# merijn-23/magr-ray-tracer

Hardware: AMD Instinct MI355X
Metric: Mrays/sec + extend-kernel HBM GB/s, sponza 1080p 256spp (higher is better)
Workload: dtype f32

## Files before the change

### include/rt355.h

```cpp
#ifndef RT355_H
#define RT355_H
#include "rt355_types.h"

#ifdef __cplusplus
extern "C" {
#endif

#define RT_OK            0
#define RT_E_INVALID    (-1)
#define RT_E_DEVICE     (-2)
#define RT_E_NOMEM      (-3)
#define RT_E_UNSUPPORTED (-4)

#define RT_SHADING_SIMPLE       0
#define RT_SHADING_NEE          1
#define RT_SAMPLING_HEMISPHERE  0
#define RT_SAMPLING_COSINE      1
#define RT_ACCEL_BVH2           0
#define RT_ACCEL_BVH4           1

typedef struct RtCtx RtCtx;

typedef struct RtConfig {
    int32_t width, height;
// ... 84 lines not shown
int rt_debug_sbvh_phases(float* out);
int rt_build_bvh4(int32_t device, const RtBVHNode2* nodes2, int32_t nNodes, int32_t nIdx, const uint32_t* roots, int32_t nRoots,
                  RtBVHNode4* out4, RtBvh4Stats* stats);

typedef struct RtUpdateStats {
    double  gpu_ms;
    int32_t prims, nodes;
    int32_t tlas_nodes, tlas_depth;
    int32_t reconfigured;
    int32_t reserved[3];
} RtUpdateStats;
int rt_update_scene(RtCtx* ctx, const RtPrimitive* prims, int32_t first, int32_t count, const RtBVHInstance* blas, int32_t nBlas,
                    RtUpdateStats* stats);
#define RT_REBUILD_SAH   0
#define RT_REBUILD_LBVH  1
#define RT_REBUILD_SBVH  2
typedef struct RtRebuildStats {
    double  gpu_ms;
    double  wall_ms;
    double  stage_ms, build_ms, derive_ms, tlas_ms, commit_ms;
    int32_t prims, blas_built;
    int32_t nodes, n_idx;
    int32_t max_depth;
    int32_t tlas_nodes, tlas_depth;
    int32_t reconfigured;
    int32_t spatial_splits, prims_clipped;
} RtRebuildStats;
int rt_rebuild_scene(RtCtx* ctx, const RtPrimitive* prims, int32_t first, int32_t count, const RtBVHInstance* blas, int32_t nBlas,
                     int32_t builder, const RtBuildOptions* opts, RtRebuildStats* stats);
int rt_debug_rebuild_allocations(RtCtx* ctx, int64_t* count);
int rt_blas_ranges(const RtBVHNode2* nodes, int32_t nNodes, const uint32_t* primIdx, int32_t nIdx, int32_t nPrims,
                   const RtBVHInstance* blas, int32_t nBlas, int32_t* firstOut, int32_t* countOut);
#define RT_SCENE_PRIMS         0
#define RT_SCENE_BVH           1
#define RT_SCENE_TLAS          2
#define RT_SCENE_INSTANCES     3
#define RT_SCENE_PAIRS         4
#define RT_SCENE_TRI_RECS      5
#define RT_SCENE_SHADE_RECS    6
#define RT_SCENE_LIGHT_RECS    7
#define RT_SCENE_TLAS_PAIRS    8
#define RT_SCENE_TLAS_PAIRS_P  9
#define RT_SCENE_INST_RECS    10
#define RT_SCENE_QUADS        11
#define RT_SCENE_ROOT_ENTRY   12
#define RT_SCENE_BVH2_KEPT    13
int rt_debug_get_scene_array(RtCtx* ctx, int32_t which, void* out, int64_t capacityBytes, int64_t* bytes);

typedef struct RtGroup RtGroup;
int rt_group_create(const RtConfig* cfg, int32_t lanes, RtGroup** out);
int rt_group_destroy(RtGroup* g);
int rt_group_lanes(RtGroup* g);
int rt_group_concurrency(RtGroup* g);
RtCtx* rt_group_lane(RtGroup* g, int32_t m);
uint64_t rt_group_frames(RtGroup* g);
int rt_group_upload_scene(RtGroup* g,
                          const RtPrimitive* prims, int32_t nPrims, const RtMaterial* mats, int32_t nMats,
                          const RtFloat4* textures, int32_t nTexels, const uint32_t* lights, int32_t nLights,
                          const void* bvhNodes, int32_t nNodes, const uint32_t* primIdx, int32_t nIdx,
                          const RtTLASNode* tlas, int32_t nTlas, const RtBVHInstance* blas, int32_t nBlas);
int rt_group_upload_scene_bvh2(RtGroup* g,
                               const RtPrimitive* prims, int32_t nPrims, const RtMaterial* mats, int32_t nMats,
                               const RtFloat4* textures, int32_t nTexels, const uint32_t* lights, int32_t nLights,
                               const RtBVHNode2* bvhNodes, int32_t nNodes, const uint32_t* primIdx, int32_t nIdx,
                               const RtTLASNode* tlas, int32_t nTlas, const RtBVHInstance* blas, int32_t nBlas);
int rt_group_share_scene(RtGroup* g, RtGroup* from);
int rt_group_update_scene(RtGroup* g, const RtPrimitive* prims, int32_t first, int32_t count, const RtBVHInstance* blas, int32_t nBlas,
                          RtUpdateStats* stats);
int rt_group_rebuild_scene(RtGroup* g, const RtPrimitive* prims, int32_t first, int32_t count, const RtBVHInstance* blas, int32_t nBlas,
                           int32_t builder, const RtBuildOptions* opts, RtRebuildStats* stats);
int rt_group_seed(RtGroup* g, uint64_t firstStream);
int rt_group_reset(RtGroup* g);
int rt_group_render(RtGroup* g, const RtCamera* cam, const RtSettings* settings, int32_t frames);
int rt_group_synchronize(RtGroup* g);
int rt_group_sum(RtGroup* g, void* devicePtr);
int rt_group_read_accum(RtGroup* g, RtFloat4* out);
int rt_group_focus(RtGroup* g, int32_t x, int32_t y, const RtCamera* cam, float* t);
int rt_group_postproc(RtGroup* g, int32_t frames, float vignette, float gamma, float chromatic, RtFloat4* outF32, uint8_t* outRGBA8);

int rt_set_seeds(RtCtx* ctx, const uint32_t* seeds, int64_t n);
int rt_seed_default(RtCtx* ctx);
int rt_get_seeds(RtCtx* ctx, uint32_t* out, int64_t n);

int rt_bind_accum(RtCtx* ctx, void* devicePtr);
void* rt_accum_device_ptr(RtCtx* ctx);
void* rt_stream(RtCtx* ctx);

int rt_reset(RtCtx* ctx);

int rt_render(RtCtx* ctx, const RtCamera* cam, const RtSettings* settings, int32_t frames);
int rt_synchronize(RtCtx* ctx);

int rt_focus(RtCtx* ctx, int32_t x, int32_t y, const RtCamera* cam, float* t);

int rt_read_accum(RtCtx* ctx, RtFloat4* out);
int rt_write_accum(RtCtx* ctx, const RtFloat4* in);
int rt_read_counters(RtCtx* ctx, RtCounters* out);
int rt_reset_counters(RtCtx* ctx);
int rt_set_profile(RtCtx* ctx, int32_t level);
int rt_read_stage_times(RtCtx* ctx, RtStageTimes* out);
int rt_reset_stage_times(RtCtx* ctx);

int rt_postproc(RtCtx* ctx, int32_t frames, float vignette, float gamma, float chromatic, RtFloat4* outF32, uint8_t* outRGBA8);

int rt_stage_begin_frame(RtCtx* ctx);
int rt_stage_generate(RtCtx* ctx, const RtCamera* cam, const RtSettings* s);
// ... 31 lines not shown
```

### magr_ray_tracer_amd/_lib.py

```python
import ctypes as C
import os

import numpy as np

_PKG = os.path.dirname(os.path.abspath(__file__))

f4 = np.dtype((np.float32, 4))
Ray = np.dtype([("O", f4), ("D", f4), ("rD", f4), ("N", f4), ("I", f4), ("intensity", f4), ("t", "<f4"),
                ("primIdx", "<i4"), ("bounces", "<i4"), ("pixelIdx", "<i4"), ("inside", "u1"), ("lastSpecular", "u1"),
                ("_pad0", "u1", 2), ("u", "<f4"), ("v", "<f4"), ("_pad1", "<u4")], align=False)
ShadowRay = np.dtype([("I", f4), ("L", f4), ("Nl", f4), ("intensity", f4), ("BRDF", f4), ("lightIdx", "<i4"),
                      ("pixelIdx", "<i4"), ("dotNL", "<f4"), ("dist", "<f4")])
Material = np.dtype([("color", f4), ("absorption", f4), ("specular", "<f4"), ("n1", "<f4"), ("n2", "<f4"),
                     ("isDielectric", "u1"), ("_pad0", "u1", 3), ("texIdx", "<i4"), ("texW", "<i4"), ("texH", "<i4"),
                     ("isLight", "u1"), ("_pad1", "u1", 3), ("emittance", f4)])
Primitive = np.dtype([("v0", f4), ("v1", f4), ("v2", f4), ("N", f4), ("centroid", f4), ("uv0", "<f4", 2), ("uv1", "<f4", 2),
                      ("uv2", "<f4", 2), ("_padt", "<f4", 2), ("objType", "<i4"), ("matIdx", "<i4"), ("area", "<f4"),
                      ("_pad", "<u4")])
Camera = np.dtype([("type", "<i4"), ("fov", "<f4"), ("aperture", "<f4"), ("focalLength", "<f4"), ("forward", f4),
                   ("right", f4), ("up", f4), ("origin", f4), ("horizontal", f4), ("vertical", f4), ("topLeft", f4)])
Settings = np.dtype([("numPrimitives", "<i4"), ("numLights", "<i4"), ("tracerType", "<i4"), ("frames", "<i4"),
                     ("antiAliasing", "<i4"), ("numInRays", "<i4"), ("numOutRays", "<i4"), ("shadowRays", "<i4"),
                     ("renderBVH", "<i4"), ("focalLength", "<f4")])
BVHNode2 = np.dtype([("aabbMin", f4), ("aabbMax", f4), ("first", "<u4"), ("count", "<u4"), ("_pad", "<u4", 2)])
# ... 21 lines not shown
                     [("sah_cost", "<f4"), ("device_ms", "<f4"), ("wall_ms", "<f4"), ("peak_refs", "<i4")])
Bvh4Stats = np.dtype([(n, "<i4") for n in ("live_nodes", "levels", "stack_need", "largest_leaf")] + [("device_ms", "<f4"), ("wall_ms", "<f4")])
KernelInfo = np.dtype([(n, "<i4") for n in ("layout", "persist", "persist4", "stack_entries", "persist_grid", "persist_grid_connect",
                                             "shade_grid", "n_blas")])

_SIZES = {"Ray": (Ray, 128), "ShadowRay": (ShadowRay, 96), "Material": (Material, 80), "Primitive": (Primitive, 128),
          "Camera": (Camera, 128), "Settings": (Settings, 40), "BVHNode2": (BVHNode2, 48), "BVHNode4": (BVHNode4, 160),
          "BVHInstance": (BVHInstance, 68), "TLASNode": (TLASNode, 48), "BuildOptions": (BuildOptions, 16), "BuildStats": (BuildStats, 32), "SbvhStats": (SbvhStats, 48), "Bvh4Stats": (Bvh4Stats, 24), "ShadowRecord": (ShadowRecord, 48), "Config": (Config, 64)}
for _n, (_d, _s) in _SIZES.items():
    assert _d.itemsize == _s, (_n, _d.itemsize, _s)

SHADING_SIMPLE, SHADING_NEE = 0, 1
SAMPLING_HEMISPHERE, SAMPLING_COSINE = 0, 1
ACCEL_BVH2, ACCEL_BVH4 = 0, 1
PRIM_SPHERE, PRIM_PLANE, PRIM_TRIANGLE = 0, 1, 2
MATH_EXP, MATH_SIN, MATH_COS, MATH_ACOS, MATH_ATAN, MATH_F2I, MATH_ATAN2, MATH_SPHERE_TEXEL, MATH_NORMALIZE4, MATH_LENGTH4 = range(10)
MATH_WORDS = {MATH_EXP: (1, 1), MATH_SIN: (1, 1), MATH_COS: (1, 1), MATH_ACOS: (1, 1), MATH_ATAN: (1, 1), MATH_F2I: (1, 1),
              MATH_ATAN2: (2, 1), MATH_SPHERE_TEXEL: (6, 2), MATH_NORMALIZE4: (4, 4), MATH_LENGTH4: (4, 1)}
MATH_SWEEP_BLOCK_BITS = 20
MAX_BOUNCES = 7
BUILTINS_DEFAULT, BUILTINS_IEEE, BUILTINS_REFERENCE = 0, 1, 2
BUILTINS = {None: BUILTINS_DEFAULT, "ieee": BUILTINS_IEEE, "reference": BUILTINS_REFERENCE}


def builtins_value(name):
    try:
        return BUILTINS[name]
    except (KeyError, TypeError):
        raise ValueError(f"builtins must be None, 'ieee' or 'reference', not {name!r}") from None


RT_OK, RT_E_INVALID, RT_E_DEVICE, RT_E_NOMEM, RT_E_UNSUPPORTED = 0, -1, -2, -3, -4
SCENE_ARRAYS = {"prims": 0, "bvh": 1, "tlas": 2, "instances": 3, "pairs": 4, "triRecs": 5, "shadeRecs": 6, "lightRecs": 7,
                "tlasPairs": 8, "tlasPairsP": 9, "instRecs": 10}
SCENE_ARRAYS_BVH4 = {"quads": 11, "rootEntry": 12, "bvh2Kept": 13}
UpdateStats = np.dtype([("gpu_ms", "<f8"), ("prims", "<i4"), ("nodes", "<i4"), ("tlas_nodes", "<i4"), ("tlas_depth", "<i4"),
                        ("reconfigured", "<i4"), ("reserved", "<i4", 3)])
assert UpdateStats.itemsize == 40
REBUILD_SAH, REBUILD_LBVH, REBUILD_SBVH = 0, 1, 2
RebuildStats = np.dtype([(n, "<f8") for n in ("gpu_ms", "wall_ms", "stage_ms", "build_ms", "derive_ms", "tlas_ms", "commit_ms")] +
                        [(n, "<i4") for n in ("prims", "blas_built", "nodes", "n_idx", "max_depth", "tlas_nodes", "tlas_depth", "reconfigured")] +
                        [("spatial_splits", "<i4"), ("prims_clipped", "<i4")])
assert RebuildStats.itemsize == 96

DEVICE_SYMBOLS = [
    "rt_last_error", "rt_device_count", "rt_kernel_info", "rt_builtins", "rt_top_levels", "rt_shade_footprint", "rt_shade_tables", "rt_create", "rt_destroy", "rt_upload_scene", "rt_share_scene", "rt_set_seeds", "rt_seed_default",
    "rt_get_seeds", "rt_bind_accum", "rt_accum_device_ptr", "rt_stream", "rt_reset", "rt_render", "rt_synchronize", "rt_focus",
    "rt_read_accum", "rt_write_accum", "rt_postproc", "rt_read_counters", "rt_reset_counters", "rt_read_stage_times", "rt_reset_stage_times", "rt_set_profile",
    "rt_stage_begin_frame", "rt_stage_generate", "rt_stage_extend", "rt_stage_shade", "rt_stage_connect",
    "rt_debug_get_rays", "rt_debug_set_rays", "rt_debug_get_shadow", "rt_debug_enable_steps", "rt_debug_get_steps", "rt_debug_math",
    "rt_debug_math_sweep", "rt_debug_math_mode", "rt_debug_math_sweep_mode", "rt_validate_scene", "rt_build_bvh2", "rt_build_bvh2_sah", "rt_debug_sah_phases", "rt_build_bvh2_sbvh", "rt_debug_sbvh_phases", "rt_update_scene", "rt_group_update_scene", "rt_debug_get_scene_array",
    "rt_rebuild_scene", "rt_group_rebuild_scene", "rt_blas_ranges", "rt_debug_rebuild_allocations",
    "rt_build_bvh4", "rt_upload_scene_bvh2", "rt_group_upload_scene_bvh2",
    "rt_group_create", "rt_group_destroy", "rt_group_lanes", "rt_group_concurrency", "rt_group_lane", "rt_group_frames", "rt_group_upload_scene", "rt_group_share_scene",
    "rt_group_seed", "rt_group_reset", "rt_group_render", "rt_group_synchronize", "rt_group_sum", "rt_group_read_accum", "rt_group_focus",
    "rt_group_postproc"]
HOST_SYMBOLS = [
    "rth_last_error", "rth_scene_create", "rth_scene_destroy", "rth_add_material", "rth_add_texture", "rth_load_texture", "rth_add_sphere",
    "rth_add_plane", "rth_add_triangle", "rth_add_quad", "rth_add_triangles", "rth_build_blas", "rth_build_bvh4",
    "rth_build_tlas", "rth_bvh4_from_nodes", "rth_set_instance_transform", "rth_primitives", "rth_materials", "rth_textures", "rth_lights",
    "rth_bvh2_nodes", "rth_bvh4_nodes", "rth_prim_idx", "rth_tlas_nodes", "rth_blas_nodes", "rth_bvh_stats", "rth_camera",
    "rth_renderer_create", "rth_renderer_destroy", "rth_renderer_init", "rth_renderer_set_camera", "rth_renderer_tick",
    "rth_renderer_read", "rth_renderer_camera", "rth_seed_stream", "rth_load_model", "rth_save_png",
    "rth_set_build_threads", "rth_renderer_save_frame", "rth_renderer_camera_move", "rth_renderer_camera_mouse", "rth_renderer_camera_zoom", "rth_renderer_frames", "rth_renderer_set_lanes", "rth_renderer_set_builtins", "rth_renderer_builtins",
    "rth_build_blas_lbvh", "rth_build_bvh2_lbvh", "rth_lbvh_stats", "rth_set_primitives", "rth_refit",
    "rth_build_blas_sah_gpu", "rth_build_bvh2_sah", "rth_build_blas_sbvh_gpu", "rth_build_bvh2_sbvh", "rth_rebuild", "rth_blas_ranges",
    "rth_build_bvh4_gpu", "rth_build_bvh4_levels"]

_dev = None
_host = None


class NativeLibraryMissing(RuntimeError):
    pass


def _load(name, local=False):
    path = os.path.join(_PKG, name)
    if not os.path.exists(path):
        raise NativeLibraryMissing(
            f"{path} is missing: build it with `python -m magr_ray_tracer_amd.build` (hipcc, gfx950). "
            "The hot path has no Python/CPU fallback.")
    return C.CDLL(path, mode=C.RTLD_LOCAL if local else C.RTLD_GLOBAL)


_variants = {}


def device_lib(variant=None):
    global _dev
    if variant:
        if variant not in _variants:
            keep, _dev = _dev, None
            try:
                _variants[variant] = _bind_device(_load(f"librt355_{variant}.so", local=True))
            finally:
                _dev = keep
        return _variants[variant]
    if _dev is None:
        _dev = _bind_device(_load("librt355.so"))
    return _dev


def _bind_device(lib):
    if True:
        vp, i32, i64 = C.c_void_p, C.c_int32, C.c_int64
        lib.rt_last_error.restype = C.c_char_p
# ... 10 lines not shown
        lib.rt_build_bvh4.argtypes = [i32, vp, i32, i32, vp, i32, vp, vp]
        lib.rt_share_scene.argtypes = [vp, vp]
        lib.rt_set_seeds.argtypes = [vp, vp, i64]
        lib.rt_seed_default.argtypes = [vp]
        lib.rt_get_seeds.argtypes = [vp, vp, i64]
        lib.rt_bind_accum.argtypes = [vp, vp]
        lib.rt_accum_device_ptr.argtypes = [vp]
        lib.rt_accum_device_ptr.restype = vp
        lib.rt_stream.argtypes = [vp]
        lib.rt_stream.restype = vp
        lib.rt_reset.argtypes = [vp]
        lib.rt_render.argtypes = [vp, vp, vp, i32]
        lib.rt_synchronize.argtypes = [vp]
        lib.rt_focus.argtypes = [vp, i32, i32, vp, C.POINTER(C.c_float)]
        lib.rt_read_accum.argtypes = [vp, vp]
        lib.rt_read_counters.argtypes = [vp, vp]
        lib.rt_write_accum.argtypes = [vp, vp]
        lib.rt_postproc.argtypes = [vp, i32, C.c_float, C.c_float, C.c_float, vp, vp]
        lib.rt_reset_counters.argtypes = [vp]
        lib.rt_read_stage_times.argtypes = [vp, vp]
        lib.rt_reset_stage_times.argtypes = [vp]
        lib.rt_set_profile.argtypes = [vp, i32]
        lib.rt_stage_begin_frame.argtypes = [vp]
        lib.rt_stage_generate.argtypes = [vp, vp, vp]
        lib.rt_stage_extend.argtypes = [vp, i32, i32]
        lib.rt_stage_shade.argtypes = [vp, i32]
        lib.rt_stage_connect.argtypes = [vp, i32, i32]
        lib.rt_debug_get_rays.argtypes = [vp, i32, vp, i32, C.POINTER(i32)]
        lib.rt_debug_set_rays.argtypes = [vp, i32, vp, i32]
        lib.rt_debug_get_shadow.argtypes = [vp, i32, i32, vp, i32, C.POINTER(i32)]
        lib.rt_debug_get_steps.argtypes = [vp, vp, i32, C.POINTER(i32)]
        lib.rt_debug_enable_steps.argtypes = [vp, i32]
        lib.rt_debug_math.argtypes = [i32, vp, vp, i64]
        lib.rt_debug_math_sweep.argtypes = [i32, i32, i32, vp]
        lib.rt_debug_math_mode.argtypes = [i32, i32, vp, vp, i64]
        lib.rt_debug_math_sweep_mode.argtypes = [i32, i32, i32, i32, vp]
        lib.rt_validate_scene.argtypes = [i32, vp, i32, vp, i32, vp, i32, vp, i32, vp, i32, vp, i32, vp, i32, vp, i32]
        lib.rt_build_bvh2.argtypes = [i32, vp, vp, i32, i32, i32, C.c_uint32, C.c_uint32, vp, i32, C.POINTER(i32), vp, vp]
        lib.rt_build_bvh2_sah.argtypes = [i32, vp, i32, i32, i32, C.c_uint32, C.c_uint32, vp, i32, C.POINTER(i32), vp, vp]
        lib.rt_debug_sah_phases.argtypes = [vp]
        lib.rt_build_bvh2_sbvh.argtypes = [i32, C.c_float, vp, i32, i32, i32, C.c_uint32, C.c_uint32, vp, i32, C.POINTER(i32), vp, i32, C.POINTER(i32), vp]
        lib.rt_debug_sbvh_phases.argtypes = [vp]
        lib.rt_update_scene.argtypes = [vp, vp, i32, i32, vp, i32, vp]
        lib.rt_group_update_scene.argtypes = [vp, vp, i32, i32, vp, i32, vp]
        lib.rt_debug_get_scene_array.argtypes = [vp, i32, vp, i64, C.POINTER(i64)]
        lib.rt_rebuild_scene.argtypes = [vp, vp, i32, i32, vp, i32, i32, vp, vp]
        lib.rt_group_rebuild_scene.argtypes = [vp, vp, i32, i32, vp, i32, i32, vp, vp]
        lib.rt_debug_rebuild_allocations.argtypes = [vp, vp]
        lib.rt_blas_ranges.argtypes = [vp, i32, vp, i32, i32, vp, i32, vp, vp]
        lib.rt_group_create.argtypes = [vp, i32, C.POINTER(vp)]
        lib.rt_group_destroy.argtypes = [vp]
        lib.rt_group_lanes.argtypes = [vp]
        lib.rt_group_concurrency.argtypes = [vp]
        lib.rt_group_lane.argtypes = [vp, i32]
        lib.rt_group_lane.restype = vp
        lib.rt_group_frames.argtypes = [vp]
        lib.rt_group_frames.restype = C.c_uint64
        lib.rt_group_upload_scene.argtypes = [vp, vp, i32, vp, i32, vp, i32, vp, i32, vp, i32, vp, i32, vp, i32, vp, i32]
        lib.rt_group_seed.argtypes = [vp, C.c_uint64]
        lib.rt_group_share_scene.argtypes = [vp, vp]
        lib.rt_group_reset.argtypes = [vp]
        lib.rt_group_render.argtypes = [vp, vp, vp, i32]
        lib.rt_group_synchronize.argtypes = [vp]
        lib.rt_group_sum.argtypes = [vp, vp]
        lib.rt_group_read_accum.argtypes = [vp, vp]
        lib.rt_group_focus.argtypes = [vp, i32, i32, vp, C.POINTER(C.c_float)]
        lib.rt_group_postproc.argtypes = [vp, i32, C.c_float, C.c_float, C.c_float, vp, vp]
    return lib


def host_lib():
    global _host
    if _host is None:
        device_lib()
        lib = _load("librt355_host.so")
        vp, i32, fp, cp = C.c_void_p, C.c_int, C.POINTER(C.c_float), C.c_char_p
        lib.rth_last_error.restype = cp
        lib.rth_scene_create.restype = vp
        lib.rth_scene_destroy.argtypes = [vp]
        lib.rth_add_material.argtypes = [vp, cp, vp]
        lib.rth_add_texture.argtypes = [vp, cp, vp, i32, i32]
        lib.rth_load_texture.argtypes = [vp, cp, cp]
        lib.rth_add_sphere.argtypes = [vp, fp, C.c_float, cp]
        lib.rth_add_plane.argtypes = [vp, fp, C.c_float, cp]
        lib.rth_add_triangle.argtypes = [vp, fp, fp, fp, fp, fp, fp, cp, i32]
        lib.rth_add_quad.argtypes = [vp, fp, fp, fp, fp, cp, i32]
        lib.rth_add_triangles.argtypes = [vp, vp, vp, i32, cp, i32]
        lib.rth_build_blas.argtypes = [vp, i32, C.c_float]
        lib.rth_build_bvh4.argtypes = [vp]
        lib.rth_build_bvh4_gpu.argtypes = [vp, i32]
        lib.rth_build_bvh4_levels.argtypes = [vp, C.c_int32, C.c_int32, vp, C.c_int32, vp, vp, vp, vp, vp]
        lib.rth_build_blas_lbvh.argtypes = [vp, i32, i32, vp]
        lib.rth_build_bvh2_lbvh.argtypes = [vp, vp, C.c_int32, C.c_int32, C.c_int32, C.c_uint32, C.c_uint32, vp, C.c_int32,
                                            C.POINTER(C.c_int32), vp, vp]
        lib.rth_lbvh_stats.argtypes = [vp, vp]
        lib.rth_build_blas_sah_gpu.argtypes = [vp, i32, i32]
        lib.rth_build_bvh2_sah.argtypes = [vp, C.c_int32, C.c_int32, C.c_int32, C.c_uint32, C.c_uint32, vp, C.c_int32,
                                           C.POINTER(C.c_int32), vp, vp]
        lib.rth_build_blas_sbvh_gpu.argtypes = [vp, i32, C.c_float, i32]
        lib.rth_build_bvh2_sbvh.argtypes = [C.c_float, vp, C.c_int32, C.c_int32, C.c_int32, C.c_uint32, C.c_uint32, vp, C.c_int32,
                                            C.POINTER(C.c_int32), vp, C.c_int32, C.POINTER(C.c_int32), vp]
        lib.rth_set_primitives.argtypes = [vp, i32, i32, vp]
        lib.rth_refit.argtypes = [vp]
        lib.rth_rebuild.argtypes = [vp, i32, vp]
        lib.rth_blas_ranges.argtypes = [vp, vp, vp]
        lib.rth_set_build_threads.argtypes = [vp, i32]
# ... 43 lines not shown
```

### magr_ray_tracer_amd/csrc/rt355.hip

```cpp
#include <hip/hip_runtime.h>
#include <hip/hip_ext.h>
#include <algorithm>
#include <chrono>
#include <cstdio>
#include <cmath>
#include <cstdlib>
#include <cstring>
#include <memory>
#include <atomic>
#include <string>
#include <vector>
#include "../../include/rt355.h"
#include "rt355_kernels.h"
#include "scene_dev.h"

using namespace rt355dev;
using namespace scenedev;

static constexpr int kAdmitAnySgpr = 6, kAdmit96Sgpr = 7;
static constexpr int kTopLevelsExtend = 6, kTopLevelsConnect = 6;
static constexpr int kFitSeven = 22, kBackupWords = 10, kSpillCap = kFitSeven - kBackupWords;
static thread_local std::string g_err;
int rt355_set_error(int code, const char* msg) { g_err = msg; return code; }

// ... 1194 lines not shown
    int rc = math_device("rt_debug_math_sweep"); if (rc) return rc;
    if (nBlocks == 0) return RT_OK;
    unsigned long long* dH = nullptr;
    hipError_t e = hipMalloc((void**)&dH, sizeof(uint64_t) * nBlocks);
    if (e == hipSuccess) e = hipMemset(dH, 0, sizeof(uint64_t) * nBlocks);
    if (e == hipSuccess) {
        const int groups = nBlocks * ((1 << RT_MATH_SWEEP_BLOCK_BITS) / (kBlock * kSweepPerThread));
        hipLaunchKernelGGL(refb ? k_debug_math_sweep<true> : k_debug_math_sweep<false>, dim3(groups), dim3(kBlock), 0, 0, (int)fn, (uint32_t)firstBlock, dH);
        e = hipGetLastError();
    }
    if (e == hipSuccess) e = hipMemcpy(hashes, dH, sizeof(uint64_t) * nBlocks, hipMemcpyDeviceToHost);
    (void)hipFree(dH);
    if (e != hipSuccess) return fail(RT_E_DEVICE, "rt_debug_math_sweep: %s", hipGetErrorString(e));
    return RT_OK;
}
extern "C" int rt_debug_math_sweep(int32_t fn, int32_t firstBlock, int32_t nBlocks, uint64_t* hashes) { return rt_debug_math_sweep_mode(RT_BUILTINS_DEFAULT, fn, firstBlock, nBlocks, hashes); }

extern "C" int rt_postproc(RtCtx* ctx, int32_t frames, float vignette, float gamma, float chromatic, RtFloat4* outF32, uint8_t* outRGBA8)
{
    if (!ctx) return fail(RT_E_INVALID, "rt_postproc: null context");
    if (frames <= 0) return fail(RT_E_INVALID, "rt_postproc: frames must be > 0 (it is the divisor of prep())");
    HIPCHK(hipSetDevice(ctx->cfg.device));
    const size_t px = (size_t)ctx->cfg.width * ctx->cfg.height;
    if (!ctx->dPostF) { HIPCHK(hipMalloc((void**)&ctx->dPostF, px * sizeof(float4))); HIPCHK(hipMalloc((void**)&ctx->dPostB, px * 4)); }
    PostParams pp{ 1 / (float)frames, vignette, gamma, chromatic, ctx->cfg.width, ctx->cfg.height };
    hipLaunchKernelGGL(k_postproc, grid_for((int)px), dim3(kBlock), 0, ctx->stream, (const float4*)ctx->q.accum, ctx->dPostF, ctx->dPostB, pp);
    HIPCHK(hipGetLastError());
    if (outF32) HIPCHK(hipMemcpyAsync(outF32, ctx->dPostF, px * sizeof(float4), hipMemcpyDeviceToHost, ctx->stream));
    if (outRGBA8) HIPCHK(hipMemcpyAsync(outRGBA8, ctx->dPostB, px * 4, hipMemcpyDeviceToHost, ctx->stream));
    HIPCHK(hipStreamSynchronize(ctx->stream));
    ev_collect(ctx);
    return RT_OK;
}


__global__ void k_spin(long long ticks, int* sink)
{
    const long long t0 = wall_clock64();
    while (wall_clock64() - t0 < ticks) __builtin_amdgcn_s_sleep(8);
    if (ticks < 0) *sink = 1;
}
__global__ __launch_bounds__(kBlock) void k_sum_lanes(float4* out, const float4* a0, const float4* a1, const float4* a2, const float4* a3,
                                                       const float4* a4, const float4* a5, const float4* a6, const float4* a7, int lanes, int first, int n)
{
    int i = blockIdx.x * kBlock + threadIdx.x;
    if (i >= n) return;
    i += first;
    const float4* a[8] = { a0, a1, a2, a3, a4, a5, a6, a7 };
    float4 s = a[0][i];
    for (int m = 1; m < lanes; m++) s = add4(s, a[m][i]);
    out[i] = s;
}

struct RtGroup {
    std::vector<RtCtx*> lane;
    float4* sum = nullptr;
    std::vector<hipEvent_t> done;
    uint64_t frames = 0;
    int concurrent = 0;
    std::vector<int> worker;
    std::vector<hipEvent_t> moved;
    int nextLane = 0;
    int nextWorker = 0;
};
static constexpr int kMaxLanes = 8;

static void group_free(RtGroup* g)
{
    if (!g) return;
    for (RtCtx* c : g->lane) { (void)hipStreamSynchronize(c->stream); c->stream = c->home; }
    for (RtCtx* c : g->lane) ctx_free(c);
    for (hipEvent_t e : g->done) (void)hipEventDestroy(e);
    for (hipEvent_t e : g->moved) (void)hipEventDestroy(e);
    if (g->sum) (void)hipFree(g->sum);
    delete g;
}
static std::vector<int> measure_workers(RtGroup* g)
{
    const int n = (int)g->lane.size();
    std::vector<int> set{ 0 };
    if (n <= 1) return set;
    int rate = 0;
    if (hipDeviceGetAttribute(&rate, hipDeviceAttributeWallClockRate, g->lane[0]->cfg.device) != hipSuccess || rate <= 0) rate = 100000;
    const long long ticks = (long long)rate;
    int* sink = (int*)g->lane[0]->q.fault;
    auto run = [&](const std::vector<int>& lanes) {
        const auto t0 = std::chrono::steady_clock::now();
        for (int m : lanes) hipLaunchKernelGGL(k_spin, dim3(1), dim3(64), 0, g->lane[(size_t)m]->home, ticks, sink);
        for (int m : lanes) (void)hipStreamSynchronize(g->lane[(size_t)m]->home);
        return std::chrono::duration<float, std::milli>(std::chrono::steady_clock::now() - t0).count();
    };
    auto best = [&](const std::vector<int>& lanes) { float t = run(lanes); for (int k = 0; k < 2; k++) t = std::min(t, run(lanes)); return t; };
    std::vector<int> all(n);
    for (int m = 0; m < n; m++) all[(size_t)m] = m;
    (void)run(all);
    const float one = best(set);
    if (one <= 0) return set;
    for (int m = 1; m < n; m++) {
        std::vector<int> cand = set; cand.push_back(m);
        if (best(cand) < 1.5f * one) set = cand;
    }
    return set;
}

extern "C" int rt_group_create(const RtConfig* cfg, int32_t lanes, RtGroup** out)
{
    if (!cfg || !out) return fail(RT_E_INVALID, "rt_group_create: null argument");
    if (lanes < 1 || lanes > kMaxLanes) return fail(RT_E_INVALID, "rt_group_create: lanes must be 1..%d", kMaxLanes);
    std::unique_ptr<RtGroup, void (*)(RtGroup*)> guard(new RtGroup(), group_free);
    RtGroup* g = guard.get();
    for (int m = 0; m < lanes; m++) {
        RtConfig c = *cfg;
        if (lanes > 1) {
            if (c.shade_blocks_per_cu == 0) c.shade_blocks_per_cu = 1;
        }
        if (m > 0) c.profile = 0;
        RtCtx* ctx = nullptr;
        const int rc = rt_create(&c, &ctx);
        if (rc != RT_OK) return rc;
        g->lane.push_back(ctx);
        for (auto* ev : { &g->done, &g->moved }) {
            hipEvent_t e;
            if (hipEventCreateWithFlags(&e, hipEventDisableTiming) != hipSuccess) return fail(RT_E_DEVICE, "rt_group_create: hipEventCreate failed");
            ev->push_back(e);
        }
    }
    const size_t px = (size_t)cfg->width * cfg->height;
    if (hipMalloc((void**)&g->sum, px * sizeof(float4)) != hipSuccess) return fail(RT_E_NOMEM, "rt_group_create: hipMalloc of the group accumulator failed");
    HIPCHK(hipMemset(g->sum, 0, px * sizeof(float4)));
    g->worker = measure_workers(g);
    if (const char* t = getenv("RT355_GROUP_STREAMS")) {
        const int k = atoi(t);
        if (k >= 1 && k < (int)g->worker.size()) g->worker.resize((size_t)k);
    }
    g->concurrent = (int)g->worker.size();
    if (lanes > 1 && cfg->persist_blocks_per_cu == 0)
        for (RtCtx* c : g->lane) c->cfg.persist_blocks_per_cu = g->concurrent >= 4 ? 2 : 3;
    if (g->concurrent < lanes) {
        static bool warned = false;
        if (!warned) {
            warned = true;
            fprintf(stderr, "librt355: %d lanes requested but only %d of their HIP streams run concurrently (GPU_MAX_HW_QUEUES=%s; HIP serialises streams that "
                            "share a hardware queue)\n",
                    lanes, g->concurrent, getenv("GPU_MAX_HW_QUEUES") ? getenv("GPU_MAX_HW_QUEUES") : "unset");
        }
    }
    *out = guard.release();
    return RT_OK;
}
extern "C" int rt_group_destroy(RtGroup* g) { group_free(g); return RT_OK; }
extern "C" int rt_group_lanes(RtGroup* g) { return g ? (int)g->lane.size() : 0; }
extern "C" int rt_group_concurrency(RtGroup* g) { return g ? g->concurrent : 0; }
extern "C" RtCtx* rt_group_lane(RtGroup* g, int32_t m) { return g && m >= 0 && m < (int)g->lane.size() ? g->lane[(size_t)m] : nullptr; }
extern "C" uint64_t rt_group_frames(RtGroup* g) { return g ? g->frames : 0; }

extern "C" int rt_group_upload_scene(RtGroup* g, const RtPrimitive* prims, int32_t nPrims, const RtMaterial* mats, int32_t nMats,
                                     const RtFloat4* textures, int32_t nTexels, const uint32_t* lights, int32_t nLights,
                                     const void* bvhNodes, int32_t nNodes, const uint32_t* primIdx, int32_t nIdx,
                                     const RtTLASNode* tlas, int32_t nTlas, const RtBVHInstance* blas, int32_t nBlas)
{
    if (!g) return fail(RT_E_INVALID, "rt_group_upload_scene: null group");
    int rc = rt_upload_scene(g->lane[0], prims, nPrims, mats, nMats, textures, nTexels, lights, nLights, bvhNodes, nNodes, primIdx, nIdx, tlas, nTlas, blas, nBlas);
    for (size_t m = 1; m < g->lane.size() && rc == RT_OK; m++) rc = rt_share_scene(g->lane[m], g->lane[0]);
    return rc;
}
extern "C" int rt_group_upload_scene_bvh2(RtGroup* g, const RtPrimitive* prims, int32_t nPrims, const RtMaterial* mats, int32_t nMats,
                                          const RtFloat4* textures, int32_t nTexels, const uint32_t* lights, int32_t nLights,
                                          const RtBVHNode2* bvhNodes, int32_t nNodes, const uint32_t* primIdx, int32_t nIdx,
                                          const RtTLASNode* tlas, int32_t nTlas, const RtBVHInstance* blas, int32_t nBlas)
{
    if (!g) return fail(RT_E_INVALID, "rt_group_upload_scene_bvh2: null group");
    int rc = rt_upload_scene_bvh2(g->lane[0], prims, nPrims, mats, nMats, textures, nTexels, lights, nLights, bvhNodes, nNodes, primIdx, nIdx, tlas, nTlas, blas, nBlas);
    for (size_t m = 1; m < g->lane.size() && rc == RT_OK; m++) rc = rt_share_scene(g->lane[m], g->lane[0]);
    return rc;
}
extern "C" int rt_group_share_scene(RtGroup* g, RtGroup* from)
{
    if (!g || !from) return fail(RT_E_INVALID, "rt_group_share_scene: null group");
    for (RtCtx* c : g->lane) { const int rc = rt_share_scene(c, from->lane[0]); if (rc != RT_OK) return rc; }
    return RT_OK;
}
extern "C" int rt_group_seed(RtGroup* g, uint64_t firstStream)
{
    if (!g) return fail(RT_E_INVALID, "rt_group_seed: null group");
    const RtCtx* c0 = g->lane[0];
    const uint64_t P = (uint64_t)c0->cfg.width * (uint64_t)c0->cfg.height;
    uint32_t x = 0x12345678u;
    auto next = [&x]() { x ^= x << 13; x ^= x >> 17; x ^= x << 5; return x; };
    uint64_t pos = 0;
    std::vector<uint32_t> s((size_t)c0->nPix);
    for (size_t m = 0; m < g->lane.size(); m++) {
        const uint64_t first = (firstStream + m) * P + (uint64_t)c0->firstPixel;
        for (; pos < first; pos++) next();
        for (auto& v : s) v = next();
        pos += s.size();
        const int rc = rt_set_seeds(g->lane[m], s.data(), (int64_t)s.size());
        if (rc != RT_OK) return rc;
    }
    return RT_OK;
}
extern "C" int rt_group_reset(RtGroup* g)
{
    if (!g) return fail(RT_E_INVALID, "rt_group_reset: null group");
    for (RtCtx* c : g->lane) { const int rc = rt_reset(c); if (rc != RT_OK) return rc; }
    g->frames = 0; g->nextLane = 0; g->nextWorker = 0;
// ... 82 lines not shown
```

### magr_ray_tracer_amd/renderer.py

```python
import ctypes as C

import numpy as np

from . import _lib


class RtError(RuntimeError):
    code = None


def _update_args(prims, first, instances):
    p = None if prims is None else np.ascontiguousarray(prims, dtype=_lib.Primitive)
    b = None if instances is None else np.ascontiguousarray(instances, dtype=_lib.BVHInstance)
    st = np.zeros((), dtype=_lib.UpdateStats)
    args = (_lib.ptr(p) if p is not None and len(p) else None, int(first), 0 if p is None else len(p),
            _lib.ptr(b) if b is not None else None, 0 if b is None else len(b), _lib.ptr(st))
    return args, (p, b), st


def _update_dict(st):
    return {"gpu_ms": float(st["gpu_ms"]), "prims": int(st["prims"]), "nodes": int(st["nodes"]), "tlas_nodes": int(st["tlas_nodes"]),
            "tlas_depth": int(st["tlas_depth"]), "reconfigured": bool(st["reconfigured"])}


# ... 266 lines not shown
        r = np.ascontiguousarray(rays, dtype=_lib.Ray)
        self._chk(self._lib.rt_debug_set_rays(self._h, bounce, _lib.ptr(r) if len(r) else _lib.ptr(np.zeros(1, dtype=_lib.Ray)), len(r)))

    def get_shadow(self, b0, b1):
        n = C.c_int32(0)
        self._chk(self._lib.rt_debug_get_shadow(self._h, b0, b1, None, 0, C.byref(n)))
        out = np.zeros(n.value, dtype=_lib.ShadowRecord)
        if n.value:
            self._chk(self._lib.rt_debug_get_shadow(self._h, b0, b1, _lib.ptr(out), n.value, C.byref(n)))
        return out

    def enable_steps(self, on=True):
        self._chk(self._lib.rt_debug_enable_steps(self._h, int(on)))

    def get_steps(self):
        n = C.c_int32(0)
        out = np.zeros(self.npix, dtype=np.int32)
        self._chk(self._lib.rt_debug_get_steps(self._h, _lib.ptr(out), out.size, C.byref(n)))
        return out


class Group:

    def __init__(self, width, height, lanes=4, y0=0, y1=None, shading=_lib.SHADING_NEE, sampling=_lib.SAMPLING_COSINE,
                 accel=_lib.ACCEL_BVH2, russian_roulette=True, filter_fireflies=True, max_bounces=_lib.MAX_BOUNCES,
                 device=0, profile=False, extend_variant=0, shade_blocks_per_cu=0, persist_blocks_per_cu=0, builtins=None):
        mode = _lib.builtins_value(builtins)
        self._lib = _lib.device_lib()
        cfg = np.zeros((), dtype=_lib.Config)
        cfg["width"], cfg["height"], cfg["y0"], cfg["y1"] = width, height, y0, height if y1 is None else y1
        cfg["max_bounces"], cfg["shading"], cfg["sampling"], cfg["accel"] = max_bounces, shading, sampling, accel
        cfg["russian_roulette"], cfg["filter_fireflies"] = int(russian_roulette), int(filter_fireflies)
        cfg["device"], cfg["profile"], cfg["extend_variant"] = device, (2 if profile is True else int(profile)), extend_variant
        cfg["shade_blocks_per_cu"], cfg["persist_blocks_per_cu"] = shade_blocks_per_cu, persist_blocks_per_cu
        cfg["builtins"] = mode
        self.cfg, self.width, self.height, self.accel = cfg, width, height, accel
        self.y0, self.y1 = int(cfg["y0"]), int(cfg["y1"])
        h = C.c_void_p()
        self._h = None
        self._chk(self._lib.rt_group_create(cfg.ctypes.data_as(C.c_void_p), int(lanes), C.byref(h)))
        self._h = h
        self.devs = [Device.borrowed(self._lib.rt_group_lane(self._h, m), cfg) for m in range(lanes)]

    def _chk(self, rc):
        if rc != 0:
            raise RtError(self._lib.rt_last_error().decode())

    def __len__(self):
        return len(self.devs)

    def concurrency(self):
        return int(self._lib.rt_group_concurrency(self._h))

    def frames(self):
        return int(self._lib.rt_group_frames(self._h))

    def upload(self, sa, from_bvh2=False):
        nodes = sa.bvh2 if from_bvh2 else sa.nodes(self.accel)
        P = _lib.ptr
        self._chk((self._lib.rt_group_upload_scene_bvh2 if from_bvh2 else self._lib.rt_group_upload_scene)(
            self._h, P(sa.prims), len(sa.prims), P(sa.mats), len(sa.mats), P(sa.tex) if len(sa.tex) else None, len(sa.tex),
            P(sa.lights) if len(sa.lights) else None, len(sa.lights), P(nodes), len(nodes), P(sa.primIdx), len(sa.primIdx),
            P(sa.tlas), len(sa.tlas), P(sa.blas), len(sa.blas)))

    def share_scene(self, other):
        self._chk(self._lib.rt_group_share_scene(self._h, other._h))

    def update_scene(self, prims=None, first=0, instances=None):
        args, keep, st = _update_args(prims, first, instances)
        self._chk(self._lib.rt_group_update_scene(self._h, *args))
        return _update_dict(st)

    def rebuild_scene(self, prims=None, first=0, instances=None, builder="sah", alpha=None, **lbvh_options):
        args, keep, st = _rebuild_args(prims, first, instances, builder, lbvh_options, alpha)
        rc = self._lib.rt_group_rebuild_scene(self._h, *args)
        if rc != 0:
            e = RtError(self._lib.rt_last_error().decode())
            e.code = rc
            raise e
        return _rebuild_dict(st)

    def seed(self, first_stream=0):
        self._chk(self._lib.rt_group_seed(self._h, int(first_stream)))

    def reset(self):
        self._chk(self._lib.rt_group_reset(self._h))

    def render(self, cam, frames=1, antiAliasing=1):
        s = np.zeros((), dtype=_lib.Settings)
        s["antiAliasing"] = antiAliasing
        c = np.ascontiguousarray(cam)
        self._chk(self._lib.rt_group_render(self._h, c.ctypes.data_as(C.c_void_p), s.ctypes.data_as(C.c_void_p), int(frames)))

    def synchronize(self):
        self._chk(self._lib.rt_group_synchronize(self._h))

    def sum_into(self, tensor):
        assert tensor.is_cuda and tensor.is_contiguous() and tensor.numel() == self.width * self.height * 4
        self._chk(self._lib.rt_group_sum(self._h, C.c_void_p(tensor.data_ptr())))

    def focus(self, x, y, cam):
        t = C.c_float(0)
        c = np.ascontiguousarray(cam)
        self._chk(self._lib.rt_group_focus(self._h, int(x), int(y), c.ctypes.data_as(C.c_void_p), C.byref(t)))
        return np.float32(t.value)

# ... 101 lines not shown
```

Measured before the change: 1034.

## Probe stream priority classes to find more concurrently running group lanes

Replaces the per-lane concurrency probe with one that measures normal, low and high priority stream classes. If the normal class does not give every lane its own hardware queue, lanes are moved onto priority streams, which get their own queue pool, so more lanes can run at once. An optional mixed mode spreads lanes across classes. This adds extra spin-kernel probing at group creation and recreates lane streams, and priority streams may be scheduled differently.

```diff
diff --git a/include/rt355.h b/include/rt355.h
--- a/include/rt355.h
+++ b/include/rt355.h
@@ -160,6 +160,8 @@
 int rt_group_destroy(RtGroup* g);
 int rt_group_lanes(RtGroup* g);
 int rt_group_concurrency(RtGroup* g);
+int rt_group_stream_class(RtGroup* g);
+int rt_group_class_concurrency(RtGroup* g, int32_t cls);
 RtCtx* rt_group_lane(RtGroup* g, int32_t m);
 uint64_t rt_group_frames(RtGroup* g);
 int rt_group_upload_scene(RtGroup* g,
diff --git a/magr_ray_tracer_amd/_lib.py b/magr_ray_tracer_amd/_lib.py
--- a/magr_ray_tracer_amd/_lib.py
+++ b/magr_ray_tracer_amd/_lib.py
@@ -97,7 +97,7 @@
     "rt_debug_math_sweep", "rt_debug_math_mode", "rt_debug_math_sweep_mode", "rt_validate_scene", "rt_build_bvh2", "rt_build_bvh2_sah", "rt_debug_sah_phases", "rt_build_bvh2_sbvh", "rt_debug_sbvh_phases", "rt_update_scene", "rt_group_update_scene", "rt_debug_get_scene_array",
     "rt_rebuild_scene", "rt_group_rebuild_scene", "rt_blas_ranges", "rt_debug_rebuild_allocations",
     "rt_build_bvh4", "rt_upload_scene_bvh2", "rt_group_upload_scene_bvh2",
-    "rt_group_create", "rt_group_destroy", "rt_group_lanes", "rt_group_concurrency", "rt_group_lane", "rt_group_frames", "rt_group_upload_scene", "rt_group_share_scene",
+    "rt_group_create", "rt_group_destroy", "rt_group_lanes", "rt_group_concurrency", "rt_group_stream_class", "rt_group_class_concurrency", "rt_group_lane", "rt_group_frames", "rt_group_upload_scene", "rt_group_share_scene",
     "rt_group_seed", "rt_group_reset", "rt_group_render", "rt_group_synchronize", "rt_group_sum", "rt_group_read_accum", "rt_group_focus",
     "rt_group_postproc"]
 HOST_SYMBOLS = [
@@ -214,6 +214,8 @@
         lib.rt_group_destroy.argtypes = [vp]
         lib.rt_group_lanes.argtypes = [vp]
         lib.rt_group_concurrency.argtypes = [vp]
+        lib.rt_group_stream_class.argtypes = [vp]
+        lib.rt_group_class_concurrency.argtypes = [vp, i32]
         lib.rt_group_lane.argtypes = [vp, i32]
         lib.rt_group_lane.restype = vp
         lib.rt_group_frames.argtypes = [vp]
diff --git a/magr_ray_tracer_amd/csrc/rt355.hip b/magr_ray_tracer_amd/csrc/rt355.hip
--- a/magr_ray_tracer_amd/csrc/rt355.hip
+++ b/magr_ray_tracer_amd/csrc/rt355.hip
@@ -1270,8 +1270,14 @@
     out[i] = s;
 }
 
+enum { kClassLow = -1, kClassNormal = 0, kClassHigh = 1, kClassMixed = 2 };
+static constexpr int kPreferClass = kClassLow;
+static constexpr bool kMixedByDefault = false;
+
 struct RtGroup {
     std::vector<RtCtx*> lane;
+    std::vector<int> laneClass;
+    int seen[3] = { -1, -1, -1 };
     float4* sum = nullptr;
     std::vector<hipEvent_t> done;
     uint64_t frames = 0;
@@ -1293,38 +1299,117 @@
     if (g->sum) (void)hipFree(g->sum);
     delete g;
 }
-static std::vector<int> measure_workers(RtGroup* g)
-{
-    const int n = (int)g->lane.size();
-    std::vector<int> set{ 0 };
-    if (n <= 1) return set;
+static std::vector<int> grow_concurrent(RtGroup* g, std::vector<hipStream_t>& set, const std::vector<hipStream_t>& cand)
+{
+    std::vector<int> taken;
+    size_t first = 0;
+    if (set.empty() && !cand.empty()) { set.push_back(cand[0]); taken.push_back(0); first = 1; }
+    if (first >= cand.size()) return taken;
     int rate = 0;
     if (hipDeviceGetAttribute(&rate, hipDeviceAttributeWallClockRate, g->lane[0]->cfg.device) != hipSuccess || rate <= 0) rate = 100000;
     const long long ticks = (long long)rate;
     int* sink = (int*)g->lane[0]->q.fault;
-    auto run = [&](const std::vector<int>& lanes) {
+    auto run = [&](const std::vector<hipStream_t>& on) {
         const auto t0 = std::chrono::steady_clock::now();
-        for (int m : lanes) hipLaunchKernelGGL(k_spin, dim3(1), dim3(64), 0, g->lane[(size_t)m]->home, ticks, sink);
-        for (int m : lanes) (void)hipStreamSynchronize(g->lane[(size_t)m]->home);
+        for (hipStream_t s : on) hipLaunchKernelGGL(k_spin, dim3(1), dim3(64), 0, s, ticks, sink);
+        for (hipStream_t s : on) (void)hipStreamSynchronize(s);
         return std::chrono::duration<float, std::milli>(std::chrono::steady_clock::now() - t0).count();
     };
-    auto best = [&](const std::vector<int>& lanes) { float t = run(lanes); for (int k = 0; k < 2; k++) t = std::min(t, run(lanes)); return t; };
-    std::vector<int> all(n);
-    for (int m = 0; m < n; m++) all[(size_t)m] = m;
+    auto best = [&](const std::vector<hipStream_t>& on) { float t = run(on); for (int k = 0; k < 2; k++) t = std::min(t, run(on)); return t; };
+    std::vector<hipStream_t> all = set;
+    all.insert(all.end(), cand.begin() + (ptrdiff_t)first, cand.end());
     (void)run(all);
-    const float one = best(set);
-    if (one <= 0) return set;
-    for (int m = 1; m < n; m++) {
-        std::vector<int> cand = set; cand.push_back(m);
-        if (best(cand) < 1.5f * one) set = cand;
-    }
-    return set;
+    const float one = best({ set[0] });
+    if (one <= 0) return taken;
+    for (size_t k = first; k < cand.size(); k++) {
+        std::vector<hipStream_t> with = set; with.push_back(cand[k]);
+        if (best(with) < 1.5f * one) { set = with; taken.push_back((int)k); }
+    }
+    return taken;
+}
+
+static int choose_streams(RtGroup* g, int want, bool mixed)
+{
+    const int n = (int)g->lane.size();
+    int least = 0, greatest = 0;
+    HIPCHK(hipDeviceGetStreamPriorityRange(&least, &greatest));
+    const bool classes = least != greatest;
+    if (!classes && (want == kClassLow || want == kClassHigh)) return fail(RT_E_INVALID, "rt_group_create: RT355_GROUP_PRIORITY asks for a priority class, but this device has one stream priority only");
+    std::vector<hipStream_t> cls[3];
+    for (RtCtx* c : g->lane) cls[1].push_back(c->home);
+    auto drop = [&](int k) { for (hipStream_t s : cls[k + 1]) if (s) (void)hipStreamDestroy(s); cls[k + 1].clear(); };
+    auto make = [&](int k) {
+        for (int m = 0; m < n; m++) {
+            hipStream_t s = nullptr;
+            const hipError_t e = hipStreamCreateWithPriority(&s, hipStreamNonBlocking, k == kClassLow ? least : greatest);
+            if (e != hipSuccess) { drop(k); return fail(RT_E_DEVICE, "rt_group_create: hipStreamCreateWithPriority failed: %s", hipGetErrorString(e)); }
+            cls[k + 1].push_back(s);
+        }
+        return (int)RT_OK;
+    };
+    std::vector<hipStream_t> set;
+    std::vector<int> worker;
+    int bestClass = kClassNormal;
+    auto measure = [&](int k) {
+        std::vector<hipStream_t> s;
+        std::vector<int> w = grow_concurrent(g, s, cls[k + 1]);
+        g->seen[k + 1] = (int)w.size();
+        if (set.empty() || w.size() > set.size() || (w.size() == set.size() && bestClass != kClassNormal && k == kPreferClass)) { set = s; worker = w; bestClass = k; }
+    };
+    if (want == kClassLow || want == kClassHigh) {
+        const int rc = make(want); if (rc != RT_OK) return rc;
+        measure(want);
+    } else {
+        measure(kClassNormal);
+        if (want != kClassNormal && classes && (int)set.size() < n)
+            for (int k : { kClassLow, kClassHigh }) {
+                const int rc = make(k); if (rc != RT_OK) { drop(kClassLow); return rc; }
+                measure(k);
+            }
+    }
+    std::vector<hipStream_t> home = cls[bestClass + 1];
+    g->laneClass.assign((size_t)n, bestClass);
+    if (mixed && classes && (int)set.size() < n) {
+        for (int m = 0; m < n; m++) {
+            if (std::find(worker.begin(), worker.end(), m) != worker.end()) continue;
+            for (int k : { kClassNormal, kClassLow, kClassHigh }) {
+                if (k == bestClass) continue;
+                if (grow_concurrent(g, set, { cls[k + 1][(size_t)m] }).empty()) continue;
+                worker.push_back(m); home[(size_t)m] = cls[k + 1][(size_t)m]; g->laneClass[(size_t)m] = k;
+                break;
+            }
+        }
+    }
+    for (int m = 0; m < n; m++) {
+        RtCtx* c = g->lane[(size_t)m];
+        for (int k = 0; k < 3; k++) if (!cls[k].empty() && cls[k][(size_t)m] == home[(size_t)m]) cls[k][(size_t)m] = nullptr;
+        if (c->home == home[(size_t)m]) continue;
+        cls[1][(size_t)m] = nullptr;
+        HIPCHK(hipStreamSynchronize(c->home));
+        HIPCHK(hipStreamDestroy(c->home));
+        c->home = c->stream = home[(size_t)m];
+    }
+    cls[1].clear();
+    drop(kClassLow); drop(kClassHigh);
+    g->worker = worker;
+    return RT_OK;
 }
 
 extern "C" int rt_group_create(const RtConfig* cfg, int32_t lanes, RtGroup** out)
 {
     if (!cfg || !out) return fail(RT_E_INVALID, "rt_group_create: null argument");
     if (lanes < 1 || lanes > kMaxLanes) return fail(RT_E_INVALID, "rt_group_create: lanes must be 1..%d", kMaxLanes);
+    int want = kClassNormal;
+    bool any = true, mixed = kMixedByDefault;
+    if (const char* t = getenv("RT355_GROUP_PRIORITY")) {
+        const std::string v(t);
+        if (v == "normal") any = false;
+        else if (v == "low") { any = false; want = kClassLow; }
+        else if (v == "high") { any = false; want = kClassHigh; }
+        else if (v == "mixed") mixed = true;
+        else if (v != "auto" && !v.empty()) return fail(RT_E_INVALID, "rt_group_create: RT355_GROUP_PRIORITY=%s is none of normal, low, high, auto, mixed", t);
+    }
+    if (!any) mixed = false;
     std::unique_ptr<RtGroup, void (*)(RtGroup*)> guard(new RtGroup(), group_free);
     RtGroup* g = guard.get();
     for (int m = 0; m < lanes; m++) {
@@ -1346,7 +1431,10 @@
     const size_t px = (size_t)cfg->width * cfg->height;
     if (hipMalloc((void**)&g->sum, px * sizeof(float4)) != hipSuccess) return fail(RT_E_NOMEM, "rt_group_create: hipMalloc of the group accumulator failed");
     HIPCHK(hipMemset(g->sum, 0, px * sizeof(float4)));
-    g->worker = measure_workers(g);
+    {
+        const int rc = choose_streams(g, any ? kClassMixed : want, mixed);
+        if (rc != RT_OK) return rc;
+    }
     if (const char* t = getenv("RT355_GROUP_STREAMS")) {
         const int k = atoi(t);
         if (k >= 1 && k < (int)g->worker.size()) g->worker.resize((size_t)k);
@@ -1358,9 +1446,12 @@
         static bool warned = false;
         if (!warned) {
             warned = true;
-            fprintf(stderr, "librt355: %d lanes requested but only %d of their HIP streams run concurrently (GPU_MAX_HW_QUEUES=%s; HIP serialises streams that "
-                            "share a hardware queue)\n",
-                    lanes, g->concurrent, getenv("GPU_MAX_HW_QUEUES") ? getenv("GPU_MAX_HW_QUEUES") : "unset");
+            static const char* const name[] = { "low", "normal", "high", "mixed" };
+            const char* q = getenv("GPU_MAX_HW_QUEUES");
+            fprintf(stderr, "librt355: %d lanes requested but only %d of their HIP streams run concurrently (stream priority class: %s; measured per class: "
+                            "low %d, normal %d, high %d, -1 = not tried; HIP serialises streams that share a hardware queue and keeps up to "
+                            "GPU_MAX_HW_QUEUES=%s of them per priority class, the normal class's shared with the process's other streams)\n",
+                    lanes, g->concurrent, name[rt_group_stream_class(g) + 1], g->seen[0], g->seen[1], g->seen[2], q ? q : "4 (unset)");
         }
     }
     *out = guard.release();
@@ -1369,6 +1460,13 @@
 extern "C" int rt_group_destroy(RtGroup* g) { group_free(g); return RT_OK; }
 extern "C" int rt_group_lanes(RtGroup* g) { return g ? (int)g->lane.size() : 0; }
 extern "C" int rt_group_concurrency(RtGroup* g) { return g ? g->concurrent : 0; }
+extern "C" int rt_group_stream_class(RtGroup* g)
+{
+    if (!g || g->laneClass.empty()) return kClassNormal;
+    for (int k : g->laneClass) if (k != g->laneClass[0]) return kClassMixed;
+    return g->laneClass[0];
+}
+extern "C" int rt_group_class_concurrency(RtGroup* g, int32_t cls) { return g && cls >= kClassLow && cls <= kClassHigh ? g->seen[cls + 1] : -1; }
 extern "C" RtCtx* rt_group_lane(RtGroup* g, int32_t m) { return g && m >= 0 && m < (int)g->lane.size() ? g->lane[(size_t)m] : nullptr; }
 extern "C" uint64_t rt_group_frames(RtGroup* g) { return g ? g->frames : 0; }
 
diff --git a/magr_ray_tracer_amd/renderer.py b/magr_ray_tracer_amd/renderer.py
--- a/magr_ray_tracer_amd/renderer.py
+++ b/magr_ray_tracer_amd/renderer.py
@@ -342,6 +342,13 @@
     def concurrency(self):
         return int(self._lib.rt_group_concurrency(self._h))
 
+    def stream_class(self):
+        return {-1: "low", 0: "normal", 1: "high", 2: "mixed"}[int(self._lib.rt_group_stream_class(self._h))]
+
+    def class_concurrency(self):
+        seen = {name: int(self._lib.rt_group_class_concurrency(self._h, k)) for k, name in ((-1, "low"), (0, "normal"), (1, "high"))}
+        return {name: s for name, s in seen.items() if s >= 0}
+
     def frames(self):
         return int(self._lib.rt_group_frames(self._h))
 
```

After: 1078, median of 6. +4.3%, better.
